# MPEGGroup/mpeg-pcc-tmc2

Hardware: AMD Instinct MI355X
Metric: encoder patch+image-gen frames/sec, longdress_vox10 32-frame GOF (higher is better)
Workload: dtype int32/f64

## Files before the change

### mpeg-pcc-tmc2_amd/csrc/api.cpp

```cpp
#include <algorithm>
#include <cstring>
#include <atomic>
#include <chrono>
#include <condition_variable>
#include <cstdarg>
#include <map>
#include <memory>
#include <mutex>

#include "internal.h"

extern char** environ;

namespace tmc2 {
int allowLargeLds( const void* kernel, size_t bytes, int device, size_t staticBytes ) {
  static std::mutex                                 lock;
  static std::map<std::pair<const void*, int>, int> granted;
  std::lock_guard<std::mutex>                       g( lock );
  int& have = granted[{kernel, device}];
  if ( int( bytes ) <= have ) return TMC2_OK;
  const int want = 160 * 1024 - int( ( staticBytes + 63 ) & ~size_t( 63 ) );
  if ( int( bytes ) > want ) {
    setError( "%zu bytes of dynamic LDS requested (+ %zu static): more than a gfx950 workgroup has", bytes, staticBytes );
    return TMC2_E_INVALID;
// ... 173 lines not shown
  (void)hipEventRecord( stages[id].pending.back().second, stream );
}
void tmc2_ctx::foldStage( StageTimer& t ) {
  for ( auto& pr : t.pending ) {
    float ms = 0.f;
    if ( hipEventSynchronize( pr.second ) == hipSuccess && hipEventElapsedTime( &ms, pr.first, pr.second ) == hipSuccess )
      t.ms += ms;
    freeEvents.push_back( pr.first );
    freeEvents.push_back( pr.second );
  }
  t.pending.clear();
}
void tmc2_ctx::stageAddHostMs( const char* name, double ms ) {
  for ( auto& s : stages )
    if ( s.name == name ) {
      s.ms += ms;
      s.calls++;
      return;
    }
  StageTimer t;
  t.name  = name;
  t.ms    = ms;
  t.calls = 1;
  stages.push_back( t );
}

extern "C" {

const char* tmc2_last_error( void ) { return g_lastError.c_str(); }

int tmc2_ctx_create( int device, tmc2_ctx** out ) {
  if ( !out ) return TMC2_E_INVALID;
  *out      = nullptr;
  int count = 0;
  if ( hipGetDeviceCount( &count ) != hipSuccess || count <= 0 ) {
    setError( "no HIP device visible: this library has no CPU path" );
    return TMC2_E_NO_DEVICE;
  }
  if ( device < 0 || device >= count ) {
    setError( "device %d out of range (%d visible)", device, count );
    return TMC2_E_INVALID;
  }
  TMC2_HIP( hipSetDevice( device ) );
  tmc2_ctx* c = new tmc2_ctx();
  c->device   = device;
  hipDeviceProp_t prop;
// ... 604 lines not shown
```

### mpeg-pcc-tmc2_amd/csrc/internal.h

```cpp
#pragma once
#include <hip/hip_runtime.h>

#include <algorithm>
#include <cstdint>
#include <cstdio>
#include <cstring>
#include <initializer_list>
#include <atomic>
#include <map>
#include <memory>
#include <mutex>
#include <optional>
#include <string>
#include <functional>
#include <vector>

#include "tmc2hip.h"

namespace tmc2 {

void setError( const char* fmt, ... );

#define TMC2_HIP( expr )                                                                        \
  do {                                                                                          \
// ... 237 lines not shown
  tmc2::DevBuf<uint32_t>        voxelBitmap;
  std::map<uint32_t, int>       kdLevelHint;
  struct ConstTable {
    tmc2::DevBuf<int> dev;
    std::vector<int>  host;
  };
  std::map<uint64_t, std::unique_ptr<ConstTable>> constTables;
  std::vector<std::unique_ptr<ConstTable>>        retiredTables;
  const int* constTable( uint64_t key, const std::vector<int>& host );
  uint32_t* mailbox = nullptr;
  static constexpr size_t kMailboxWords = 1024;
  volatile uint32_t* answerLine( int line ) const { return mailbox + size_t( line ) * 16; }
  enum { kAnswerRefineVoxels = 1, kAnswerPatchRound = 2, kAnswerRecon = 3, kAnswerOrientHead = 4, kAnswerTreeDepth = 5, kAnswerGeoError = 6, kAnswerAttrError = 7, kAnswerTreeLevels = 8 , kAnswerVoxelCount = 13 };
  std::map<std::string, std::string> options;
  mutable std::mutex                 optionsLock;
  std::shared_ptr<tmc2_host_gate>    hostGate;
  hipStream_t                   stream = nullptr;
  std::vector<tmc2::StageTimer> stages;
  std::vector<hipEvent_t>       freeEvents;
  bool                          timing = true;
  int                           cuCount = 256;
  void foldStage( tmc2::StageTimer& t );
  void stageAddHostMs( const char* name, double ms );

 private:
  friend struct tmc2::StageScope;
  int  stageBegin( const char* name );
  void stageEnd( int id );
};

namespace tmc2 {
struct StageScope {
  StageScope( tmc2_ctx* c, const char* name ) : ctx( c ), id( c->stageBegin( name ) ) {}
  StageScope( const StageScope& ) = delete;
  StageScope& operator=( const StageScope& ) = delete;
  ~StageScope() { end(); }
  void end() { ctx->stageEnd( id ), id = -1; }

 private:
  tmc2_ctx* ctx;
  int       id;
};
void destroyContextNow( tmc2_ctx* ctx );
struct FrameTicket {
  tmc2_ctx* ctx = nullptr;
  void      bind( tmc2_ctx* c ) {
// ... 207 lines not shown
```

### mpeg-pcc-tmc2_amd/csrc/kdtree_device.hip

```cpp
#include <algorithm>
#include <cstring>

#include "internal.h"

namespace tmc2 {
namespace {

constexpr uint32_t kNone      = 0xFFFFFFFFu;
constexpr int      kBlock     = 256;
constexpr int      kWaves     = kBlock / 64;
constexpr int      kScanTile  = kBlock * 8;
constexpr int      kLeafMax   = 10;
constexpr int      kMaxLevels = 64;

struct BuildSeg {
  uint32_t begin, end;
  uint32_t node, parent;
  int32_t  mn[3], mx[3];
  int16_t  lo[3], hi[3];
  uint8_t  side, pdim;
  uint8_t  split, cutDim;
  int32_t  cut;
  uint32_t mid;
  uint32_t slot;
};

struct RetiredSeg {
  uint32_t begin, end, node, level;
  int16_t  lo[3], hi[3];
  int32_t  root;
};

struct HugeSeg {
  uint32_t begin, end, node, level;
  int16_t  lo[3], hi[3];
  int32_t  root;
  int32_t  mn[3], mx[3];
};

struct BuildArgs {
  const Pt* pts;
  uint32_t  n, tiles;
  Pt*       P;
  uint32_t *perm, *seg;
  BuildSeg *segA, *segB;
  KdNode*   nodes;
  uint32_t *loc1, *loc2, *tile1, *tile2;
  uint32_t* counts;
  uint32_t* nodeCount;
  int32_t*  rootBox;
  uint32_t* levels;
  RetiredSeg* retired;
  uint32_t*   retiredCount;
  uint32_t*   bigCount;
  HugeSeg*    huge;
  uint32_t*   hugeCount;
  uint32_t    hugeMax;
  uint32_t    retireMax, splitMax;
  struct LvSeg *lvA, *lvB;
  uint16_t*   list;
  struct LvPartial* partial;
  unsigned long long* pieceProfile;
  uint32_t    decideRng;
  uint32_t*   finishDepth;
  uint32_t*   ticket;
  volatile uint32_t* hostSmall;
  volatile uint32_t* hostDepth;
};

__device__ __forceinline__ int coordOf( const Pt p, int d ) { return d == 0 ? p.x : ( d == 1 ? p.y : p.z ); }

struct SplitRule {
  int     dim;
  int32_t cut;
};
__device__ __forceinline__ SplitRule splitOf( const int16_t ( &lo )[3], const int16_t ( &hi )[3], const int32_t ( &mn )[3],
                                              const int32_t ( &mx )[3] ) {
  const int32_t maxSpan = max( int32_t( hi[0] ) - lo[0], max( int32_t( hi[1] ) - lo[1], int32_t( hi[2] ) - lo[2] ) );
  SplitRule     r;
  r.dim              = 0;
  int32_t bestSpread = -1;
#pragma unroll
  for ( int d = 0; d < 3; ++d ) {
    if ( double( int32_t( hi[d] ) - lo[d] ) > ( 1.0 - 0.00001 ) * double( maxSpan ) ) {
      const int32_t spread = mx[d] - mn[d];
      if ( spread > bestSpread ) {
        bestSpread = spread;
        r.dim      = d;
      }
    }
  }
// ... 166 lines not shown
          child[0].begin = q.begin, child[0].end = q.begin + idx, child[0].node = id0;
          child[1].begin = q.begin + idx, child[1].end = q.end, child[1].node = id0 + 1;
          for ( int c = 0; c < 2; ++c ) {
            child[c].depth = uint16_t( q.depth + 1 );
            for ( int d = 0; d < 3; ++d )
              child[c].lo[d] = lo[d], child[c].hi[d] = hi[d], child[c].mn[d] = int16_t( r[6 * c + d] ), child[c].mx[d] = int16_t( r[6 * c + 3 + d] );
          }
          const int16_t cut = int16_t( rule.cut );
          if ( rule.dim == 0 ) child[0].hi[0] = cut, child[1].lo[0] = cut;
          if ( rule.dim == 1 ) child[0].hi[1] = cut, child[1].lo[1] = cut;
          if ( rule.dim == 2 ) child[0].hi[2] = cut, child[1].lo[2] = cut;
          for ( int c = 0; c < 2; ++c ) {
            const uint32_t cc = child[c].end - child[c].begin, level = seg.level + child[c].depth;
            if ( cc <= uint32_t( kLeafMax ) ) {
              KdNode leaf;
              leaf.a = int32_t( seg.begin + child[c].begin ), leaf.b = int32_t( seg.begin + child[c].end ), leaf.divlow = leaf.divhigh = 0,
              leaf.dim = -1;
              a.nodes[child[c].node] = leaf;
              atomicMax( a.finishDepth, level + 1u );
            } else if ( cc <= a.retireMax ) {
              RetiredSeg rs;
              rs.begin = seg.begin + child[c].begin, rs.end = seg.begin + child[c].end, rs.node = child[c].node, rs.level = level, rs.root = 0;
              for ( int d = 0; d < 3; ++d ) rs.lo[d] = child[c].lo[d], rs.hi[d] = child[c].hi[d];
              a.retired[atomicAdd( a.retiredCount, 1u )] = rs;
            } else {
              sNode[cur ^ 1][sCount[cur ^ 1]++] = child[c];
            }
          }
        }
        __syncthreads();
      }
      if ( threadIdx.x == 0 ) sCount[cur] = 0;
      cur ^= 1;
      __syncthreads();
    }
  }
}

constexpr int      kPieceMax  = 4096;
constexpr int      kPieceRecs = kPieceMax / ( kLeafMax + 1 ) + 2;
constexpr uint16_t kNoRec     = 0xFFFFu;
constexpr uint32_t kNoKey     = 0xFFFFFFFFu;

struct alignas( 8 ) PieceRec {
  uint16_t begin, end;
  int16_t  cut;
  uint8_t  dim, unused0;
  uint16_t edge1, rb1;
  uint16_t edge2, rb2;
  uint16_t mid;
  uint16_t child[2];
  uint16_t unused1;
  uint32_t node;
  int32_t  lmax, rmin;
  int16_t  lo[3], hi[3];
  int32_t  mn[3], mx[3];
};
static_assert( sizeof( PieceRec ) == 72, "PieceRec layout" );
struct PieceHot0 {
  uint32_t be, dc;
};
struct PieceHot1 {
  uint32_t e1rb1, e2rb2;
// ... 115 lines not shown
  }
#pragma unroll
  for ( int off = 32; off > 0; off >>= 1 ) {
    mnx = min( mnx, __shfl_xor( mnx, off, 64 ) ), mny = min( mny, __shfl_xor( mny, off, 64 ) ), mnz = min( mnz, __shfl_xor( mnz, off, 64 ) );
    mxx = max( mxx, __shfl_xor( mxx, off, 64 ) ), mxy = max( mxy, __shfl_xor( mxy, off, 64 ) ), mxz = max( mxz, __shfl_xor( mxz, off, 64 ) );
  }
  if ( lane == 0 ) {
    int* w = blockRange + 6 * wave;
    w[0] = mnx, w[1] = mny, w[2] = mnz, w[3] = mxx, w[4] = mxy, w[5] = mxz;
  }
  __syncthreads();
  if ( threadIdx.x < 6 ) {
    int v = blockRange[threadIdx.x];
    for ( int w = 1; w < kWaves; ++w ) v = threadIdx.x < 3 ? min( v, blockRange[6 * w + threadIdx.x] ) : max( v, blockRange[6 * w + threadIdx.x] );
    int32_t* slot = threadIdx.x < 3 ? &a.lvA[0].mn[threadIdx.x] : &a.lvA[0].mx[threadIdx.x - 3];
    if ( threadIdx.x < 3 ) {
      if ( v < loadStaleOk( slot ) ) atomicMin( slot, v );
    } else {
      if ( v > loadStaleOk( slot ) ) atomicMax( slot, v );
    }
  }
}
__global__ void lvRootKernel( BuildArgs a ) {
  if ( threadIdx.x < kMaxLevels + 16 ) a.counts[threadIdx.x] = 0;
  __syncthreads();
  if ( threadIdx.x != 0 ) return;
  LvSeg r{};
  r.begin = 0, r.end = a.n, r.node = 0, r.parent = kNone;
  for ( int d = 0; d < 3; ++d ) r.mn[d] = 0x7FFFFFFF, r.mx[d] = int32_t( 0x80000000 );
  a.lvA[0]     = r;
  a.counts[0]  = 1;
  *a.nodeCount = 1;
}

constexpr int kDecideThreads = 1024;
constexpr int kDecideRng     = 2000;
__global__ __launch_bounds__( kDecideThreads ) void lvDecideKernel( BuildArgs a, uint32_t level ) {
  __shared__ uint32_t waveTot[kDecideThreads / 64];
  __shared__ uint32_t sCarry;
  __shared__ int32_t  sRng[kDecideRng][6];
  LvSeg*         cur   = ( level & 1 ) ? a.lvB : a.lvA;
  const uint32_t count = a.counts[level], nodeBase = *a.nodeCount;
  const int      lane = threadIdx.x & 63, wave = threadIdx.x >> 6;
  if ( threadIdx.x == 0 ) sCarry = 0;
  const bool inLds = level > 0 && count <= a.decideRng;
  if ( inLds ) {
    for ( uint32_t t = threadIdx.x; t < count * 6u; t += kDecideThreads ) sRng[t / 6u][t % 6u] = ( t % 6u ) < 3u ? 0x7FFFFFFF : int32_t( 0x80000000 );
// ... 37 lines not shown
        if ( inLds ) mn[d] = min( mn[d], sRng[s][d] ), mx[d] = max( mx[d], sRng[s][3 + d] );
        lo[d] = root ? mn[d] : int32_t( q->lo[d] );
        hi[d] = root ? mx[d] : int32_t( q->hi[d] );
      }
      if ( root ) {
        for ( int d = 0; d < 3; ++d ) a.rootBox[d] = mn[d], a.rootBox[3 + d] = mx[d];
      } else {
        const int pd = q->pdim;
        if ( q->side == 0 )
          a.nodes[q->parent].divlow = int16_t( pd == 0 ? mx[0] : ( pd == 1 ? mx[1] : mx[2] ) );
        else
          a.nodes[q->parent].divhigh = int16_t( pd == 0 ? mn[0] : ( pd == 1 ? mn[1] : mn[2] ) );
      }
      const uint32_t cnt = q->end - q->begin;
      if ( cnt <= uint32_t( kLeafMax ) ) {
        KdNode nd;
        nd.a = int32_t( q->begin ), nd.b = int32_t( q->end ), nd.divlow = nd.divhigh = 0, nd.dim = -1;
        a.nodes[q->node] = nd;
      } else if ( cnt <= a.retireMax ) {
        RetiredSeg r;
        r.begin = q->begin, r.end = q->end, r.node = q->node, r.level = level;
        r.root  = root ? 1 : 0;
        for ( int d = 0; d < 3; ++d ) r.lo[d] = q->lo[d], r.hi[d] = q->hi[d];
        a.retired[atomicAdd( a.retiredCount, 1u )] = r;
      } else if ( cnt <= a.hugeMax ) {
        HugeSeg r;
        r.begin = q->begin, r.end = q->end, r.node = q->node, r.level = level;
        r.root  = root ? 1 : 0;
        for ( int d = 0; d < 3; ++d ) r.lo[d] = q->lo[d], r.hi[d] = q->hi[d], r.mn[d] = mn[d], r.mx[d] = mx[d];
        a.huge[atomicAdd( a.hugeCount, 1u )] = r;
      } else {
        const int32_t maxSpan = max( hi[0] - lo[0], max( hi[1] - lo[1], hi[2] - lo[2] ) );
        const double  limit   = ( 1.0 - 0.00001 ) * double( maxSpan );
        int           dim     = 0;
        int32_t       best    = -1;
        if ( double( hi[0] - lo[0] ) > limit && mx[0] - mn[0] > best ) best = mx[0] - mn[0], dim = 0;
        if ( double( hi[1] - lo[1] ) > limit && mx[1] - mn[1] > best ) best = mx[1] - mn[1], dim = 1;
        if ( double( hi[2] - lo[2] ) > limit && mx[2] - mn[2] > best ) best = mx[2] - mn[2], dim = 2;
        const int32_t l = dim == 0 ? lo[0] : ( dim == 1 ? lo[1] : lo[2] ), h = dim == 0 ? hi[0] : ( dim == 1 ? hi[1] : hi[2] );
        const int32_t lowest = dim == 0 ? mn[0] : ( dim == 1 ? mn[1] : mn[2] ), highest = dim == 0 ? mx[0] : ( dim == 1 ? mx[1] : mx[2] );
        const int32_t cut = min( max( ( l + h ) / 2, lowest ), highest );
        q->cutInfo = ( uint32_t( cut ) & 0xFFFFu ) | ( uint32_t( dim ) << 16 ) | ( 1u << 24 );
        if ( root )
          for ( int d = 0; d < 3; ++d ) q->lo[d] = int16_t( mn[d] ), q->hi[d] = int16_t( mx[d] );
        split = 1;
      }
      if ( !split ) q->cutInfo = 0;
// ... 4 lines not shown
      const uint32_t t = __shfl_up( inc, off, 64 );
      if ( lane >= off ) inc += t;
    }
    if ( lane == 63 ) waveTot[wave] = inc;
    __syncthreads();
    uint32_t before = sCarry, all = 0;
    for ( int w = 0; w < kDecideThreads / 64; ++w ) {
      all += waveTot[w];
      before += w < wave ? waveTot[w] : 0u;
    }
    const uint32_t rank = before + inc - split;
    if ( split ) q->slot = 2u * rank, q->childNode = nodeBase + 2u * rank;
    __syncthreads();
    if ( threadIdx.x == 0 ) sCarry += all;
    __syncthreads();
  }
  if ( threadIdx.x == 0 ) {
    a.counts[level + 1] = 2u * sCarry;
    *a.nodeCount        = nodeBase + 2u * sCarry;
  }
  if ( a.hostSmall ) {
    if ( threadIdx.x == 0 ) __threadfence();
    __syncthreads();
    if ( threadIdx.x < kMaxLevels + 16 ) a.hostSmall[threadIdx.x] = __hip_atomic_load( &a.counts[threadIdx.x], __ATOMIC_RELAXED, __HIP_MEMORY_SCOPE_AGENT );
  }
}

template <bool FIRST>
__global__ __launch_bounds__( kBlock ) void lvFlagKernel( BuildArgs a, uint32_t level ) {
  __shared__ uint32_t waveSum[kWaves];
  const uint32_t n = a.n, tiles = a.tiles;
  const int      lane = threadIdx.x & 63, wave = threadIdx.x >> 6;
  LvSeg*         cur   = ( level & 1 ) ? a.lvB : a.lvA;
  LvSeg*         next  = ( level & 1 ) ? a.lvA : a.lvB;
  const uint32_t count = a.counts[level];
  uint32_t*      loc   = FIRST ? a.loc1 : a.loc2;
  uint32_t*      tile  = FIRST ? a.tile1 : a.tile2;
  if ( !FIRST ) {
    for ( uint32_t s = blockIdx.x * blockDim.x + threadIdx.x; s < count; s += gridDim.x * blockDim.x ) {
      const LvSeg* q = cur + s;
      if ( !( q->cutInfo >> 24 ) ) continue;
      for ( int c = 0; c < 2; ++c )
        for ( int d = 0; d < 3; ++d ) next[q->slot + c].mn[d] = 0x7FFFFFFF, next[q->slot + c].mx[d] = int32_t( 0x80000000 );
    }
  }
  for ( uint32_t t = blockIdx.x; t < tiles; t += gridDim.x ) {
    const uint32_t base = t * kScanTile + threadIdx.x * 8;
// ... 210 lines not shown
          }
          for ( int k = 0; k < 6; ++k ) accV[k] = accSlot == kNone ? x[k] : ( ( k % 3 ) == 1 ? pkMax( accV[k], x[k] ) : pkMin( accV[k], x[k] ) );
          accSlot = slot;
        }
      }
      __syncthreads();
      continue;
    }
    if ( moved ) lvReport( next + slot + 1u, pkLo( A2 ), pkHi( A2 ), pkLo( C2 ), pkLo( A2 ), pkHi( A2 ), pkLo( C2 ) );
    if ( waveSegMinMaxPacked( key, A, B, C, lane ) )
      lvReport( next + key, pkLo( A ), pkHi( A ), pkLo( C ), pkLo( B ), pkHi( B ), ~pkHi( C ) );
  }
  __syncthreads();
  if ( threadIdx.x == 0 ) {
    LvPartial pt;
    pt.slot = accSlot, pt.unused = 0;
    for ( int k = 0; k < 6; ++k ) pt.v[k] = accV[k];
    a.partial[c0 / kChunk] = pt;
  }
  __syncthreads();
  }
}

constexpr size_t kPieceLdsBytes = size_t( kPieceMax ) * ( sizeof( Pt ) + 4 + 2 + 2 + 2 ) + 16 + 2 * size_t( kPieceRecs ) * sizeof( PieceRec );

constexpr int kPiecePer = 4;
template <bool PROFILE = false>
__global__ __launch_bounds__( kPieceMax / kPiecePer ) void pieceKernel( BuildArgs a ) {
  unsigned long long profLast = 0, prof[12] = {0, 0, 0, 0, 0, 0, 0, 0, 0, 0, 0, 0};
#define PIECE_MARK( k )                                        \
  if ( PROFILE && threadIdx.x == 0 ) {                         \
    const unsigned long long now_ = wall_clock64();            \
    prof[k] += now_ - profLast, profLast = now_;               \
  }
  constexpr int K = kPiecePer, THREADS = kPieceMax / K, WAVES = THREADS / 64;
  extern __shared__ __align__( 16 ) unsigned char pieceLds[];
  Pt*       P     = reinterpret_cast<Pt*>( pieceLds );
  uint32_t* perm  = reinterpret_cast<uint32_t*>( P + kPieceMax );
  uint16_t* pre   = reinterpret_cast<uint16_t*>( perm + kPieceMax );
  uint16_t* lst   = pre + kPieceMax + 8;
  uint16_t* segOf = lst + kPieceMax;
  PieceRec* recs  = reinterpret_cast<PieceRec*>( segOf + kPieceMax );
  __shared__ __align__( 16 ) uint32_t sWave[2][WAVES];
  __shared__ uint32_t sCount[2], sNodeBase, sDepth;
  const int      lane = threadIdx.x & 63, tid = threadIdx.x;
  const uint32_t total = *a.retiredCount;
  const uint32_t p0    = uint32_t( tid ) * K;
  for ( uint32_t s = blockIdx.x; s < total; s += gridDim.x ) {
    const RetiredSeg seg = a.retired[s];
    const uint32_t   cnt = seg.end - seg.begin;
    uint32_t idPending   = 0;
    if ( tid == 0 ) idPending = atomicAdd( a.nodeCount, 2u );
    pieceBarrier();
    for ( uint32_t i = tid; i < uint32_t( kPieceMax ); i += THREADS ) {
      if ( i < cnt ) {
        P[i]     = a.P[seg.begin + i];
        perm[i]  = a.perm[seg.begin + i];
        segOf[i] = 0;
      } else {
        segOf[i] = kNoRec;
      }
    }
    if ( tid == 0 ) {
      PieceRec r{};
      r.begin = 0, r.end = uint16_t( cnt ), r.node = seg.node;
      for ( int d = 0; d < 3; ++d ) r.lo[d] = seg.lo[d], r.hi[d] = seg.hi[d], r.mn[d] = 0x7FFFFFFF, r.mx[d] = int32_t( 0x80000000 );
      recs[0]   = r;
      sCount[0] = 1, sCount[1] = 0, sDepth = 0;
    }
    pieceBarrier();
    {
      uint32_t A = pk2( 0x7FFF, 0x7FFF ), B = pk2( -0x8000, -0x8000 ), C = pk2( 0x7FFF, 0x7FFF );
      bool     any = false;
#pragma unroll
      for ( int k = 0; k < K; ++k ) {
        const uint32_t p = p0 + k;
        if ( p < cnt ) {
// ... 2 lines not shown
          any = true;
        }
      }
      if ( waveSegMinMaxPacked( any ? 0u : kNoKey, A, B, C, lane ) ) {
        ldsMin( &recs[0].mn[0], pkLo( A ) ), ldsMin( &recs[0].mn[1], pkHi( A ) ), ldsMin( &recs[0].mn[2], pkLo( C ) );
        ldsMax( &recs[0].mx[0], pkLo( B ) ), ldsMax( &recs[0].mx[1], pkHi( B ) ), ldsMax( &recs[0].mx[2], ~pkHi( C ) );
      }
    }
    pieceBarrier();
    if ( seg.root != 0 && tid == 0 ) {
      for ( int d = 0; d < 3; ++d ) {
        recs[0].lo[d] = int16_t( recs[0].mn[d] ), recs[0].hi[d] = int16_t( recs[0].mx[d] );
        a.rootBox[d] = recs[0].mn[d], a.rootBox[3 + d] = recs[0].mx[d];
      }
    }
    if ( PROFILE && threadIdx.x == 0 ) profLast = wall_clock64();
    uint32_t deepest  = 0;
    uint32_t prevBase = 0, prevCount = 0;
    int      cur      = 0;
    for ( uint32_t depth = 0;; ++depth ) {
      pieceBarrier();
      PIECE_MARK( 0 )
      const uint32_t nc = sCount[cur];
      PieceRec*      R  = recs + cur * kPieceRecs;
      PieceRec*      RN = recs + ( cur ^ 1 ) * kPieceRecs;
      for ( uint32_t r = tid; r < prevCount; r += THREADS ) {
        const PieceRec* q = RN + r;
        KdNode          nd;
        nd.a = int32_t( prevBase + 2u * r ), nd.b = int32_t( prevBase + 2u * r + 1u ), nd.divlow = int16_t( q->lmax ), nd.divhigh = int16_t( q->rmin ),
        nd.dim = q->dim;
        a.nodes[q->node] = nd;
      }
      if ( nc == 0 ) break;
      if ( seg.level + depth >= uint32_t( kMaxLevels ) - 2u ) {
        if ( tid == 0 ) atomicMax( a.finishDepth, 0x10000u );
        break;
      }
      if ( tid == 0 ) sNodeBase = idPending, sCount[cur ^ 1] = 0;
      for ( uint32_t r = tid; r < nc; r += THREADS ) {
        PieceRec*     q   = R + r;
        const int32_t lo0 = q->lo[0], lo1 = q->lo[1], lo2 = q->lo[2], hi0 = q->hi[0], hi1 = q->hi[1], hi2 = q->hi[2];
        const int32_t mn0 = q->mn[0], mn1 = q->mn[1], mn2 = q->mn[2], mx0 = q->mx[0], mx1 = q->mx[1], mx2 = q->mx[2];
        const int32_t maxSpan = max( hi0 - lo0, max( hi1 - lo1, hi2 - lo2 ) );
        const double  limit   = ( 1.0 - 0.00001 ) * double( maxSpan );
        int           dim     = 0;
        int32_t       best    = -1;
        if ( double( hi0 - lo0 ) > limit && mx0 - mn0 > best ) best = mx0 - mn0, dim = 0;
        if ( double( hi1 - lo1 ) > limit && mx1 - mn1 > best ) best = mx1 - mn1, dim = 1;
// ... 27 lines not shown
          }
        }
      }
      uint32_t f1 = 0;
      if ( waveLive ) {
        Pt x[K];
#pragma unroll
        for ( int k = 0; k < K; k += 2 ) *reinterpret_cast<uint4*>( &x[k] ) = *reinterpret_cast<const uint4*>( P + p0 + k );
#pragma unroll
        for ( int k = 0; k < K; ++k ) {
          const int d = int( ( dc[k] >> 16 ) & 0xFFu ), c = int( int16_t( dc[k] & 0xFFFFu ) );
          const int v = int( int16_t( __builtin_bit_cast( uint64_t, x[k] ) >> ( 16 * d ) ) );
          if ( rec[k] != kNoRec && v >= c ) f1 |= 1u << k;
        }
      }
      uint32_t preA[K + 1];
      {
        uint32_t at = pieceScan<WAVES>( uint32_t( __popc( f1 ) ), sWave[0] );
        uint16_t out[K];
#pragma unroll
        for ( int k = 0; k < K; ++k ) preA[k] = at, out[k] = uint16_t( at ), at += ( f1 >> k ) & 1u;
        preA[K] = at;
        *reinterpret_cast<uint2*>( pre + p0 ) = *reinterpret_cast<const uint2*>( out );
        if ( tid == THREADS - 1 ) pre[kPieceMax] = uint16_t( at );
      }
      pieceBarrier();
      PIECE_MARK( 2)
      uint32_t edge1[K], rb1[K];
#pragma unroll
      for ( int k = 0; k < K; ++k ) {
        edge1[k] = rb1[k] = 0;
        if ( !waveLive || rec[k] == kNoRec ) continue;
        if ( k > 0 && rec[k] == rec[k - 1] ) {
          edge1[k] = edge1[k - 1], rb1[k] = rb1[k - 1];
        } else {
          const uint32_t b = be[k] & 0xFFFFu, e = be[k] >> 16, rb = pre[b], re = pre[e];
          edge1[k] = b + ( ( e - b ) - ( re - rb ) ), rb1[k] = rb | ( re << 16 );
        }
        const uint32_t p = p0 + k, b = be[k] & 0xFFFFu, e = be[k] >> 16;
        if ( p >= edge1[k] && !( ( f1 >> k ) & 1u ) ) lst[b + ( ( e - p - 1u ) - ( ( rb1[k] >> 16 ) - preA[k + 1] ) )] = uint16_t( p );
        if ( p == b ) *reinterpret_cast<uint32_t*>( &R[rec[k]].edge1 ) = edge1[k] | ( ( rb1[k] & 0xFFFFu ) << 16 );
      }
      pieceBarrier();
      PIECE_MARK( 3)
#pragma unroll
      for ( int k = 0; k < K; ++k ) {
        const uint32_t p = p0 + k;
// ... 5 lines not shown
        }
      }
      pieceBarrier();
      PIECE_MARK( 4)
      uint32_t f2 = 0;
      if ( waveLive ) {
        Pt x[K];
#pragma unroll
        for ( int k = 0; k < K; k += 2 ) *reinterpret_cast<uint4*>( &x[k] ) = *reinterpret_cast<const uint4*>( P + p0 + k );
#pragma unroll
        for ( int k = 0; k < K; ++k ) {
          const int d = int( ( dc[k] >> 16 ) & 0xFFu ), c = int( int16_t( dc[k] & 0xFFFFu ) );
          const int v = int( int16_t( __builtin_bit_cast( uint64_t, x[k] ) >> ( 16 * d ) ) );
          if ( rec[k] != kNoRec && p0 + k >= edge1[k] && v > c ) f2 |= 1u << k;
        }
      }
      {
        uint32_t at = pieceScan<WAVES>( uint32_t( __popc( f2 ) ), sWave[1] );
        uint16_t out[K];
#pragma unroll
        for ( int k = 0; k < K; ++k ) preA[k] = at, out[k] = uint16_t( at ), at += ( f2 >> k ) & 1u;
        preA[K] = at;
        *reinterpret_cast<uint2*>( pre + p0 ) = *reinterpret_cast<const uint2*>( out );
        if ( tid == THREADS - 1 ) pre[kPieceMax] = uint16_t( at );
      }
      pieceBarrier();
      PIECE_MARK( 5)
      const uint32_t base = sNodeBase;
      for ( uint32_t r = tid; r < nc; r += THREADS ) {
        PieceRec*      q  = R + r;
        const uint32_t b = q->begin, e = q->end, e1 = q->edge1, rb2 = pre[e1], re2 = pre[e];
        const uint32_t e2   = e1 + ( ( e - e1 ) - ( re2 - rb2 ) );
        const uint32_t n    = e - b, half = n / 2, lim1 = e1 - b, lim2 = e2 - b;
        const uint32_t idx  = lim1 > half ? lim1 : ( lim2 < half ? lim2 : half );
        const uint32_t mid  = b + idx;
        const uint32_t id0  = base + 2u * r;
        const int      dim  = q->dim;
        const int16_t  cut  = q->cut;
        q->edge2 = uint16_t( e2 ), q->rb2 = uint16_t( rb2 ), q->mid = uint16_t( mid );
        q->lmax = int32_t( 0x80000000 ), q->rmin = 0x7FFFFFFF;
#pragma unroll
        for ( int c = 0; c < 2; ++c ) {
          const uint32_t cb = c ? mid : b, ce = c ? e : mid;
          if ( ce - cb <= uint32_t( kLeafMax ) ) {
            KdNode leaf;
            leaf.a = int32_t( seg.begin + cb ), leaf.b = int32_t( seg.begin + ce ), leaf.divlow = leaf.divhigh = 0, leaf.dim = -1;
            a.nodes[id0 + c] = leaf;
// ... 134 lines not shown
  const uint32_t n = uint32_t( n64 );
  tree.n           = n64;
  tree.depth       = 0;
  for ( int d = 0; d < 3; ++d ) tree.lo[d] = tree.hi[d] = 0;
  if ( n == 0 ) return TMC2_OK;
  hipStream_t    s       = ctx->stream;
  const uint32_t tiles   = ( n + kScanTile - 1 ) / kScanTile;
  const size_t   maxSegs = 2 * ( size_t( n ) / ( kLeafMax + 1 ) + 1 ) + 2;
  const size_t   maxNode = 2 * size_t( n ) + 2;
  TMC2_TRY( tree.ptsTree.alloc( n ) );
  TMC2_TRY( tree.perm.alloc( n ) );
  TMC2_TRY( tree.nodes.alloc( maxNode ) );
  DevBuf<uint32_t>   d_work, d_small;
  DevBuf<BuildSeg>   d_segs;
  DevBuf<RetiredSeg> d_retired;
  const size_t       maxRetired = size_t( n ) / ( kLeafMax + 1 ) + 2;
  TMC2_TRY( d_retired.alloc( maxRetired ) );
  DevBuf<HugeSeg> d_huge;
  TMC2_TRY( d_huge.alloc( size_t( n ) / ( kPieceMax + 1 ) + 2 ) );
  const auto     hugeEnv = ctxOption( ctx, "KD_HUGEMAX" );
  const uint32_t hugeMax = std::min<uint32_t>( kHugeLimit, std::max<uint32_t>( kPieceMax, hugeEnv ? uint32_t( atoi( hugeEnv->c_str() ) ) : 16384u ) );
  TMC2_TRY( d_work.alloc( 3 * size_t( n ) + 2 * ( size_t( tiles ) + 1 ) ) );
  TMC2_TRY( d_segs.alloc( 2 * maxSegs ) );
  TMC2_TRY( d_small.alloc( kMaxLevels + 16 ) );
  static_assert( kMaxLevels + 16 <= 128, "lvRootKernel clears the counters with one workgroup of 128" );
  BuildArgs a;
  a.pts = d_pts, a.n = n, a.tiles = tiles, a.P = tree.ptsTree.p, a.perm = tree.perm.p;
  a.seg = d_work.p, a.loc1 = d_work.p + n, a.loc2 = d_work.p + 2 * size_t( n );
  a.tile1 = d_work.p + 3 * size_t( n ), a.tile2 = a.tile1 + tiles + 1;
  a.segA = d_segs.p, a.segB = d_segs.p + maxSegs, a.nodes = tree.nodes.p;
  a.counts    = d_small.p;
  a.nodeCount = d_small.p + kMaxLevels + 1;
  a.levels    = d_small.p + kMaxLevels + 2;
  a.rootBox   = reinterpret_cast<int32_t*>( d_small.p + kMaxLevels + 8 );
  a.retired      = d_retired.p;
  a.retiredCount = d_small.p + kMaxLevels + 3;
  a.finishDepth  = d_small.p + kMaxLevels + 4;
  a.ticket       = d_small.p + kMaxLevels + 5;
  a.bigCount     = d_small.p + kMaxLevels + 6;
  a.huge         = d_huge.p;
  a.hugeCount    = d_small.p + kMaxLevels + 7;
  a.hugeMax      = hugeMax;
  a.hostSmall    = nullptr;
  a.hostDepth    = ctx->answerLine( tmc2_ctx::kAnswerTreeDepth );
  a.retireMax    = uint32_t( kPieceMax );
  a.splitMax     = uint32_t( kPieceMax );
  const dim3 blk( kBlock ), grdE( std::max<uint32_t>( 1u, ( n + 2 * kBlock - 1 ) / ( 2 * kBlock ) ) ), grdT( tiles );
  const dim3 grdL( std::max<uint32_t>( 1u, ( n + kLandBlock * kLandRounds - 1 ) / ( kLandBlock * kLandRounds ) ) );
  const size_t sumsLds = ( size_t( tiles ) + 1 ) * 4;
  if ( sumsLds > 48 * 1024 ) {
    setError( "kdtree: %u points -- the level passes hold one word per 2 048-point tile in LDS (at most 25 M points)", n );
    return TMC2_E_UNSUPPORTED;
  }
  DevBuf<LvSeg>    d_lv;
  DevBuf<uint16_t> d_list;
  DevBuf<LvPartial> d_partial;
  const size_t     maxLv = 2 * ( size_t( n ) / ( size_t( kPieceMax ) + 1 ) + 2 );
  TMC2_TRY( d_lv.alloc( 2 * maxLv ) );
  TMC2_TRY( d_list.alloc( size_t( tiles ) * kScanTile ) );
  TMC2_TRY( d_partial.alloc( size_t( n ) / ( kLandBlock * kLandRounds ) + 2 ) );
  a.lvA = d_lv.p, a.lvB = d_lv.p + maxLv, a.list = d_list.p, a.partial = d_partial.p;
  const auto decideOpt = ctxOption( ctx, "KD_DECIDE" );
  a.decideRng = decideOpt && ( *decideOpt )[0] == 'g' ? 0u : uint32_t( kDecideRng );
  hipLaunchKernelGGL( lvRootKernel, dim3( 1 ), dim3( 128 ), 0, s, a );
  hipLaunchKernelGGL( lvInitKernel, dim3( std::min<uint32_t>( grdE.x, 1024u ) ), blk, 0, s, a );
  hipLaunchKernelGGL( lvDecideKernel, dim3( 1 ), dim3( kDecideThreads ), 0, s, a, 0u );
  uint32_t out[kMaxLevels + 16];
  int      found = -1;
  int& hint = ctx->kdLevelHint[( n >> 15 ) * 2u + 1u];
  for ( uint32_t level = 0; level < uint32_t( kMaxLevels ) && found < 0; ) {
    uint32_t chunkEnd = level + 1;
    if ( level == 0 && hint > 0 ) {
      chunkEnd = uint32_t( std::min( hint, kMaxLevels ) );
    } else {
      while ( chunkEnd < uint32_t( kMaxLevels ) && ( uint64_t( hugeMax ) << std::min<uint32_t>( chunkEnd - 1, 40 ) ) < n ) ++chunkEnd;
      if ( chunkEnd == level + 1 ) chunkEnd = std::min<uint32_t>( level + 2, kMaxLevels );
    }
    volatile uint32_t* hostSmall = ctx->answerLine( tmc2_ctx::kAnswerTreeLevels );
    for ( ; level < chunkEnd; ++level ) {
      hipLaunchKernelGGL( lvFlagKernel<true>, grdT, blk, 0, s, a, level );
      hipLaunchKernelGGL( lvSwapOneKernel, grdE, blk, sumsLds, s, a, level );
      hipLaunchKernelGGL( lvFlagKernel<false>, grdT, blk, 0, s, a, level );
      hipLaunchKernelGGL( lvSwapTwoKernel, grdL, dim3( kLandBlock ), sumsLds, s, a, level );
      BuildArgs ad = a;
      if ( level + 1 == chunkEnd ) ad.hostSmall = hostSmall;
      hipLaunchKernelGGL( lvDecideKernel, dim3( 1 ), dim3( kDecideThreads ), 0, s, ad, level + 1u );
    }
    TMC2_HIP( hipGetLastError() );
    TMC2_HIP( hipStreamSynchronize( s ) );
    for ( int w = 0; w < kMaxLevels + 16; ++w ) out[w] = hostSmall[w];
    for ( uint32_t l = 0; l <= level && l <= uint32_t( kMaxLevels ); ++l )
      if ( out[l] == 0 ) {
        found = int( l );
        break;
      }
  }
  if ( found < 0 ) {
    setError( "kdtree: more than %d levels", kMaxLevels - 1 );
    return TMC2_E_UNSUPPORTED;
  }
  tree.depth = found;
  hint       = std::max( found, 1 );
  const int32_t* box = reinterpret_cast<const int32_t*>( out + kMaxLevels + 8 );
  for ( int d = 0; d < 3; ++d ) tree.lo[d] = box[d], tree.hi[d] = box[3 + d];
  const uint32_t hugeSegs = out[kMaxLevels + 7];
  if ( hugeSegs )
    hipLaunchKernelGGL( hugeSegmentsKernel, dim3( std::min<uint32_t>( hugeSegs, 4u * uint32_t( ctx->cuCount ) ) ), dim3( 64 * kHugeWaves ), 0, s, a );
  const uint32_t retired = out[kMaxLevels + 3] + hugeSegs * ( 2u * hugeMax / uint32_t( kPieceMax ) );
  if ( retired ) {
    const dim3 grid( std::min<uint32_t>( retired, 8u * uint32_t( ctx->cuCount ) ) ), block( kPieceMax / kPiecePer );
    if ( ctxOption( ctx, "KD_PIECE_PROFILE" ) ) {
      DevBuf<unsigned long long> d_prof;
      TMC2_TRY( d_prof.alloc( 16 ) );
      TMC2_HIP( hipMemsetAsync( d_prof.p, 0, 16 * 8, s ) );
      a.pieceProfile = d_prof.p;
      TMC2_TRY( allowLargeLds( reinterpret_cast<const void*>( pieceKernel<true> ), kPieceLdsBytes, ctx->device, 256 ) );
      hipLaunchKernelGGL( pieceKernel<true>, grid, block, kPieceLdsBytes, s, a );
      unsigned long long h[16];
      TMC2_HIP( hipMemcpyAsync( h, d_prof.p, sizeof( h ), hipMemcpyDeviceToHost, s ) );
      TMC2_HIP( hipStreamSynchronize( s ) );
      static const char* what[8] = {"landing of the previous depth", "node records + split rules", "first flags + prefix sum", "first publish",
                                    "first swaps", "second flags + prefix sum", "children + second publish", "second swaps"};
      fprintf( stderr, "pieceKernel: %llu pieces, us per piece between the barriers of its depths (thread 0 of each workgroup):", h[8] );
      for ( int k = 0; k < 8; ++k ) fprintf( stderr, " %s %.1f |", what[k], 0.01 * double( h[k] ) / double( std::max<unsigned long long>( h[8], 1 ) ) );
      fprintf( stderr, "\n" );
    } else {
      TMC2_TRY( allowLargeLds( reinterpret_cast<const void*>( pieceKernel<> ), kPieceLdsBytes, ctx->device, 256 ) );
      hipLaunchKernelGGL( pieceKernel<>, grid, block, kPieceLdsBytes, s, a );
    }
    TMC2_HIP( hipGetLastError() );
    TMC2_HIP( hipStreamSynchronize( s ) );
    const uint32_t fin = *a.hostDepth;
    if ( fin >= uint32_t( kMaxLevels ) ) {
      setError( "kdtree: more than %d levels", kMaxLevels - 1 );
      return TMC2_E_UNSUPPORTED;
    }
    tree.depth = std::max( tree.depth, int( fin ) );
  }
  return TMC2_OK;
}

}
```

Baseline: 198.9.

## Bin retired kd-tree pieces by size and launch per-capacity piece kernels

Retired segments are now sorted into three size classes (up to 1024, 2048 and 4096 points). Each class gets its own pieceKernel instantiation, sized so that smaller classes use less LDS and fewer threads, which lets two or four workgroups share a CU. Workgroups take pieces through an atomic ticket instead of a grid-stride loop. The aim is to stop small pieces from occupying a full 4096-capacity workgroup and to balance work dynamically. The cost is extra kernel launches, a class-list buffer, and more atomics per piece.

```diff
diff --git a/mpeg-pcc-tmc2_amd/csrc/api.cpp b/mpeg-pcc-tmc2_amd/csrc/api.cpp
--- a/mpeg-pcc-tmc2_amd/csrc/api.cpp
+++ b/mpeg-pcc-tmc2_amd/csrc/api.cpp
@@ -219,6 +219,17 @@
   t.name  = name;
   t.ms    = ms;
   t.calls = 1;
+  stages.push_back( t );
+}
+void tmc2_ctx::stageAddCalls( const char* name, long calls ) {
+  for ( auto& s : stages )
+    if ( s.name == name ) {
+      s.calls += calls;
+      return;
+    }
+  StageTimer t;
+  t.name  = name;
+  t.calls = calls;
   stages.push_back( t );
 }
 
diff --git a/mpeg-pcc-tmc2_amd/csrc/internal.h b/mpeg-pcc-tmc2_amd/csrc/internal.h
--- a/mpeg-pcc-tmc2_amd/csrc/internal.h
+++ b/mpeg-pcc-tmc2_amd/csrc/internal.h
@@ -283,6 +283,7 @@
   int                           cuCount = 256;
   void foldStage( tmc2::StageTimer& t );
   void stageAddHostMs( const char* name, double ms );
+  void stageAddCalls( const char* name, long calls );
 
  private:
   friend struct tmc2::StageScope;
diff --git a/mpeg-pcc-tmc2_amd/csrc/kdtree_device.hip b/mpeg-pcc-tmc2_amd/csrc/kdtree_device.hip
--- a/mpeg-pcc-tmc2_amd/csrc/kdtree_device.hip
+++ b/mpeg-pcc-tmc2_amd/csrc/kdtree_device.hip
@@ -12,6 +12,17 @@
 constexpr int      kScanTile  = kBlock * 8;
 constexpr int      kLeafMax   = 10;
 constexpr int      kMaxLevels = 64;
+constexpr int      kPieceMax  = 4096;
+constexpr int      kPieceClasses = 3;
+constexpr int      kSmallHost  = kMaxLevels + 16;
+constexpr int      kSmallWords = kMaxLevels + 24;
+enum : int {
+  kWordNodeCount = kMaxLevels + 1, kWordRetired, kWordFinishDepth, kWordTicket, kWordHugeCount,
+  kWordClassCount,
+  kWordRootBox     = kSmallHost - 6,
+  kWordClassTicket = kSmallHost
+};
+static_assert( kWordClassCount + kPieceClasses <= kWordRootBox && kWordClassTicket + kPieceClasses <= kSmallWords, "counter block" );
 
 struct BuildSeg {
   uint32_t begin, end;
@@ -49,10 +60,12 @@
   uint32_t* counts;
   uint32_t* nodeCount;
   int32_t*  rootBox;
-  uint32_t* levels;
   RetiredSeg* retired;
   uint32_t*   retiredCount;
-  uint32_t*   bigCount;
+  uint32_t*   classCount;
+  uint32_t*   classList;
+  uint32_t    classStride;
+  uint32_t*   classTicket;
   HugeSeg*    huge;
   uint32_t*   hugeCount;
   uint32_t    hugeMax;
@@ -67,6 +80,14 @@
   volatile uint32_t* hostSmall;
   volatile uint32_t* hostDepth;
 };
+
+__device__ __forceinline__ void retirePiece( const BuildArgs& a, const RetiredSeg& r ) {
+  const uint32_t at = atomicAdd( a.retiredCount, 1u );
+  a.retired[at]     = r;
+  const uint32_t cnt = r.end - r.begin;
+  const int      c   = cnt <= uint32_t( kPieceMax >> 2 ) ? 0 : ( cnt <= uint32_t( kPieceMax >> 1 ) ? 1 : 2 );
+  a.classList[size_t( c ) * a.classStride + atomicAdd( a.classCount + c, 1u )] = at;
+}
 
 __device__ __forceinline__ int coordOf( const Pt p, int d ) { return d == 0 ? p.x : ( d == 1 ? p.y : p.z ); }
 
@@ -279,7 +300,7 @@
               RetiredSeg rs;
               rs.begin = seg.begin + child[c].begin, rs.end = seg.begin + child[c].end, rs.node = child[c].node, rs.level = level, rs.root = 0;
               for ( int d = 0; d < 3; ++d ) rs.lo[d] = child[c].lo[d], rs.hi[d] = child[c].hi[d];
-              a.retired[atomicAdd( a.retiredCount, 1u )] = rs;
+              retirePiece( a, rs );
             } else {
               sNode[cur ^ 1][sCount[cur ^ 1]++] = child[c];
             }
@@ -294,8 +315,7 @@
   }
 }
 
-constexpr int      kPieceMax  = 4096;
-constexpr int      kPieceRecs = kPieceMax / ( kLeafMax + 1 ) + 2;
+constexpr int pieceRecs( int cap ) { return cap / ( kLeafMax + 1 ) + 2; }
 constexpr uint16_t kNoRec     = 0xFFFFu;
 constexpr uint32_t kNoKey     = 0xFFFFFFFFu;
 
@@ -457,7 +477,7 @@
   }
 }
 __global__ void lvRootKernel( BuildArgs a ) {
-  if ( threadIdx.x < kMaxLevels + 16 ) a.counts[threadIdx.x] = 0;
+  if ( threadIdx.x < kSmallWords ) a.counts[threadIdx.x] = 0;
   __syncthreads();
   if ( threadIdx.x != 0 ) return;
   LvSeg r{};
@@ -541,7 +561,7 @@
         r.begin = q->begin, r.end = q->end, r.node = q->node, r.level = level;
         r.root  = root ? 1 : 0;
         for ( int d = 0; d < 3; ++d ) r.lo[d] = q->lo[d], r.hi[d] = q->hi[d];
-        a.retired[atomicAdd( a.retiredCount, 1u )] = r;
+        retirePiece( a, r );
       } else if ( cnt <= a.hugeMax ) {
         HugeSeg r;
         r.begin = q->begin, r.end = q->end, r.node = q->node, r.level = level;
@@ -592,7 +612,7 @@
   if ( a.hostSmall ) {
     if ( threadIdx.x == 0 ) __threadfence();
     __syncthreads();
-    if ( threadIdx.x < kMaxLevels + 16 ) a.hostSmall[threadIdx.x] = __hip_atomic_load( &a.counts[threadIdx.x], __ATOMIC_RELAXED, __HIP_MEMORY_SCOPE_AGENT );
+    if ( threadIdx.x < kSmallHost ) a.hostSmall[threadIdx.x] = __hip_atomic_load( &a.counts[threadIdx.x], __ATOMIC_RELAXED, __HIP_MEMORY_SCOPE_AGENT );
   }
 }
 
@@ -849,37 +869,48 @@
   }
 }
 
-constexpr size_t kPieceLdsBytes = size_t( kPieceMax ) * ( sizeof( Pt ) + 4 + 2 + 2 + 2 ) + 16 + 2 * size_t( kPieceRecs ) * sizeof( PieceRec );
+constexpr size_t pieceLdsBytes( int cap ) { return size_t( cap ) * ( sizeof( Pt ) + 4 + 2 + 2 + 2 ) + 16 + 2 * size_t( pieceRecs( cap ) ) * sizeof( PieceRec ); }
+constexpr size_t kCuLdsBytes = 160 * 1024, kPieceStatic = 256;
+static_assert( pieceLdsBytes( kPieceMax ) + kPieceStatic <= kCuLdsBytes, "a piece of kPieceMax points fits a CU" );
+static_assert( 2 * ( pieceLdsBytes( kPieceMax >> 1 ) + kPieceStatic ) <= kCuLdsBytes, "two workgroups of the 2 048 instance per CU" );
+static_assert( 4 * ( pieceLdsBytes( kPieceMax >> 2 ) + kPieceStatic ) <= kCuLdsBytes, "four workgroups of the 1 024 instance per CU" );
 
 constexpr int kPiecePer = 4;
-template <bool PROFILE = false>
-__global__ __launch_bounds__( kPieceMax / kPiecePer ) void pieceKernel( BuildArgs a ) {
+template <int CAP, bool PROFILE = false>
+__global__ __launch_bounds__( CAP / kPiecePer ) void pieceKernel( BuildArgs a ) {
+  static_assert( CAP == kPieceMax || CAP == kPieceMax >> 1 || CAP == kPieceMax >> 2, "one instance per capacity class" );
+  constexpr int CLS = CAP == kPieceMax ? 2 : ( CAP == kPieceMax >> 1 ? 1 : 0 ), RECS = pieceRecs( CAP );
   unsigned long long profLast = 0, prof[12] = {0, 0, 0, 0, 0, 0, 0, 0, 0, 0, 0, 0};
 #define PIECE_MARK( k )                                        \
   if ( PROFILE && threadIdx.x == 0 ) {                         \
     const unsigned long long now_ = wall_clock64();            \
     prof[k] += now_ - profLast, profLast = now_;               \
   }
-  constexpr int K = kPiecePer, THREADS = kPieceMax / K, WAVES = THREADS / 64;
+  constexpr int K = kPiecePer, THREADS = CAP / K, WAVES = THREADS / 64;
+  static_assert( WAVES % 4 == 0, "pieceScan reads the wavefront totals four at a time" );
   extern __shared__ __align__( 16 ) unsigned char pieceLds[];
   Pt*       P     = reinterpret_cast<Pt*>( pieceLds );
-  uint32_t* perm  = reinterpret_cast<uint32_t*>( P + kPieceMax );
-  uint16_t* pre   = reinterpret_cast<uint16_t*>( perm + kPieceMax );
-  uint16_t* lst   = pre + kPieceMax + 8;
-  uint16_t* segOf = lst + kPieceMax;
-  PieceRec* recs  = reinterpret_cast<PieceRec*>( segOf + kPieceMax );
+  uint32_t* perm  = reinterpret_cast<uint32_t*>( P + CAP );
+  uint16_t* pre   = reinterpret_cast<uint16_t*>( perm + CAP );
+  uint16_t* lst   = pre + CAP + 8;
+  uint16_t* segOf = lst + CAP;
+  PieceRec* recs  = reinterpret_cast<PieceRec*>( segOf + CAP );
   __shared__ __align__( 16 ) uint32_t sWave[2][WAVES];
-  __shared__ uint32_t sCount[2], sNodeBase, sDepth;
+  __shared__ uint32_t sCount[2], sNodeBase, sDepth, sPiece;
   const int      lane = threadIdx.x & 63, tid = threadIdx.x;
-  const uint32_t total = *a.retiredCount;
+  const uint32_t total = a.classCount[CLS];
+  const uint32_t* mine = a.classList + size_t( CLS ) * a.classStride;
   const uint32_t p0    = uint32_t( tid ) * K;
-  for ( uint32_t s = blockIdx.x; s < total; s += gridDim.x ) {
-    const RetiredSeg seg = a.retired[s];
+  for ( ;; ) {
+    if ( tid == 0 ) sPiece = atomicAdd( a.classTicket + CLS, 1u );
+    pieceBarrier();
+    const uint32_t t = sPiece;
+    if ( t >= total ) break;
+    const RetiredSeg seg = a.retired[mine[t]];
     const uint32_t   cnt = seg.end - seg.begin;
     uint32_t idPending   = 0;
     if ( tid == 0 ) idPending = atomicAdd( a.nodeCount, 2u );
-    pieceBarrier();
-    for ( uint32_t i = tid; i < uint32_t( kPieceMax ); i += THREADS ) {
+    for ( uint32_t i = tid; i < uint32_t( CAP ); i += THREADS ) {
       if ( i < cnt ) {
         P[i]     = a.P[seg.begin + i];
         perm[i]  = a.perm[seg.begin + i];
@@ -928,8 +959,8 @@
       pieceBarrier();
       PIECE_MARK( 0 )
       const uint32_t nc = sCount[cur];
-      PieceRec*      R  = recs + cur * kPieceRecs;
-      PieceRec*      RN = recs + ( cur ^ 1 ) * kPieceRecs;
+      PieceRec*      R  = recs + cur * RECS;
+      PieceRec*      RN = recs + ( cur ^ 1 ) * RECS;
       for ( uint32_t r = tid; r < prevCount; r += THREADS ) {
         const PieceRec* q = RN + r;
         KdNode          nd;
@@ -1003,7 +1034,7 @@
         for ( int k = 0; k < K; ++k ) preA[k] = at, out[k] = uint16_t( at ), at += ( f1 >> k ) & 1u;
         preA[K] = at;
         *reinterpret_cast<uint2*>( pre + p0 ) = *reinterpret_cast<const uint2*>( out );
-        if ( tid == THREADS - 1 ) pre[kPieceMax] = uint16_t( at );
+        if ( tid == THREADS - 1 ) pre[CAP] = uint16_t( at );
       }
       pieceBarrier();
       PIECE_MARK( 2)
@@ -1055,7 +1086,7 @@
         for ( int k = 0; k < K; ++k ) preA[k] = at, out[k] = uint16_t( at ), at += ( f2 >> k ) & 1u;
         preA[K] = at;
         *reinterpret_cast<uint2*>( pre + p0 ) = *reinterpret_cast<const uint2*>( out );
-        if ( tid == THREADS - 1 ) pre[kPieceMax] = uint16_t( at );
+        if ( tid == THREADS - 1 ) pre[CAP] = uint16_t( at );
       }
       pieceBarrier();
       PIECE_MARK( 5)
@@ -1236,24 +1267,28 @@
   const uint32_t hugeMax = std::min<uint32_t>( kHugeLimit, std::max<uint32_t>( kPieceMax, hugeEnv ? uint32_t( atoi( hugeEnv->c_str() ) ) : 16384u ) );
   TMC2_TRY( d_work.alloc( 3 * size_t( n ) + 2 * ( size_t( tiles ) + 1 ) ) );
   TMC2_TRY( d_segs.alloc( 2 * maxSegs ) );
-  TMC2_TRY( d_small.alloc( kMaxLevels + 16 ) );
-  static_assert( kMaxLevels + 16 <= 128, "lvRootKernel clears the counters with one workgroup of 128" );
+  TMC2_TRY( d_small.alloc( kSmallWords ) );
+  static_assert( kSmallWords <= 128, "lvRootKernel clears the counters with one workgroup of 128" );
+  DevBuf<uint32_t> d_classList;
+  TMC2_TRY( d_classList.alloc( size_t( kPieceClasses ) * maxRetired ) );
   BuildArgs a;
   a.pts = d_pts, a.n = n, a.tiles = tiles, a.P = tree.ptsTree.p, a.perm = tree.perm.p;
   a.seg = d_work.p, a.loc1 = d_work.p + n, a.loc2 = d_work.p + 2 * size_t( n );
   a.tile1 = d_work.p + 3 * size_t( n ), a.tile2 = a.tile1 + tiles + 1;
   a.segA = d_segs.p, a.segB = d_segs.p + maxSegs, a.nodes = tree.nodes.p;
   a.counts    = d_small.p;
-  a.nodeCount = d_small.p + kMaxLevels + 1;
-  a.levels    = d_small.p + kMaxLevels + 2;
-  a.rootBox   = reinterpret_cast<int32_t*>( d_small.p + kMaxLevels + 8 );
+  a.nodeCount = d_small.p + kWordNodeCount;
+  a.rootBox   = reinterpret_cast<int32_t*>( d_small.p + kWordRootBox );
   a.retired      = d_retired.p;
-  a.retiredCount = d_small.p + kMaxLevels + 3;
-  a.finishDepth  = d_small.p + kMaxLevels + 4;
-  a.ticket       = d_small.p + kMaxLevels + 5;
-  a.bigCount     = d_small.p + kMaxLevels + 6;
+  a.retiredCount = d_small.p + kWordRetired;
+  a.classCount   = d_small.p + kWordClassCount;
+  a.classList    = d_classList.p;
+  a.classStride  = uint32_t( maxRetired );
+  a.classTicket  = d_small.p + kWordClassTicket;
+  a.finishDepth  = d_small.p + kWordFinishDepth;
+  a.ticket       = d_small.p + kWordTicket;
   a.huge         = d_huge.p;
-  a.hugeCount    = d_small.p + kMaxLevels + 7;
+  a.hugeCount    = d_small.p + kWordHugeCount;
   a.hugeMax      = hugeMax;
   a.hostSmall    = nullptr;
   a.hostDepth    = ctx->answerLine( tmc2_ctx::kAnswerTreeDepth );
@@ -1279,7 +1314,7 @@
   hipLaunchKernelGGL( lvRootKernel, dim3( 1 ), dim3( 128 ), 0, s, a );
   hipLaunchKernelGGL( lvInitKernel, dim3( std::min<uint32_t>( grdE.x, 1024u ) ), blk, 0, s, a );
   hipLaunchKernelGGL( lvDecideKernel, dim3( 1 ), dim3( kDecideThreads ), 0, s, a, 0u );
-  uint32_t out[kMaxLevels + 16];
+  uint32_t out[kSmallHost];
   int      found = -1;
   int& hint = ctx->kdLevelHint[( n >> 15 ) * 2u + 1u];
   for ( uint32_t level = 0; level < uint32_t( kMaxLevels ) && found < 0; ) {
@@ -1302,7 +1337,7 @@
     }
     TMC2_HIP( hipGetLastError() );
     TMC2_HIP( hipStreamSynchronize( s ) );
-    for ( int w = 0; w < kMaxLevels + 16; ++w ) out[w] = hostSmall[w];
+    for ( int w = 0; w < kSmallHost; ++w ) out[w] = hostSmall[w];
     for ( uint32_t l = 0; l <= level && l <= uint32_t( kMaxLevels ); ++l )
       if ( out[l] == 0 ) {
         found = int( l );
@@ -1315,21 +1350,48 @@
   }
   tree.depth = found;
   hint       = std::max( found, 1 );
-  const int32_t* box = reinterpret_cast<const int32_t*>( out + kMaxLevels + 8 );
+  const int32_t* box = reinterpret_cast<const int32_t*>( out + kWordRootBox );
   for ( int d = 0; d < 3; ++d ) tree.lo[d] = box[d], tree.hi[d] = box[3 + d];
-  const uint32_t hugeSegs = out[kMaxLevels + 7];
+  const uint32_t hugeSegs = out[kWordHugeCount];
   if ( hugeSegs )
     hipLaunchKernelGGL( hugeSegmentsKernel, dim3( std::min<uint32_t>( hugeSegs, 4u * uint32_t( ctx->cuCount ) ) ), dim3( 64 * kHugeWaves ), 0, s, a );
-  const uint32_t retired = out[kMaxLevels + 3] + hugeSegs * ( 2u * hugeMax / uint32_t( kPieceMax ) );
-  if ( retired ) {
-    const dim3 grid( std::min<uint32_t>( retired, 8u * uint32_t( ctx->cuCount ) ) ), block( kPieceMax / kPiecePer );
-    if ( ctxOption( ctx, "KD_PIECE_PROFILE" ) ) {
-      DevBuf<unsigned long long> d_prof;
+  uint32_t classGrid[kPieceClasses];
+  int      lastClass = -1;
+  for ( int c = 0; c < kPieceClasses; ++c ) {
+    const uint32_t cap = uint32_t( kPieceMax ) >> ( kPieceClasses - 1 - c ), above = c == 0 ? uint32_t( kLeafMax ) : cap / 2u;
+    const uint64_t most = uint64_t( out[kWordClassCount + c] ) + uint64_t( hugeSegs ) * ( hugeMax / ( above + 1u ) );
+    const uint32_t resident = uint32_t( ctx->cuCount ) * ( uint32_t( kPieceMax ) / cap );
+    classGrid[c] = uint32_t( std::min<uint64_t>( most, resident ) );
+    if ( classGrid[c] && lastClass < 0 ) lastClass = c;
+  }
+  if ( lastClass >= 0 ) {
+    const bool profile = ctxOption( ctx, "KD_PIECE_PROFILE" ).has_value();
+    DevBuf<unsigned long long> d_prof;
+    if ( profile ) {
       TMC2_TRY( d_prof.alloc( 16 ) );
       TMC2_HIP( hipMemsetAsync( d_prof.p, 0, 16 * 8, s ) );
       a.pieceProfile = d_prof.p;
-      TMC2_TRY( allowLargeLds( reinterpret_cast<const void*>( pieceKernel<true> ), kPieceLdsBytes, ctx->device, 256 ) );
-      hipLaunchKernelGGL( pieceKernel<true>, grid, block, kPieceLdsBytes, s, a );
+    }
+    for ( int c = kPieceClasses - 1; c >= 0; --c ) {
+      if ( !classGrid[c] ) continue;
+      BuildArgs ac = a;
+      if ( c != lastClass ) ac.hostDepth = nullptr;
+      const dim3 grid( classGrid[c] );
+#define TMC2_PIECE_LAUNCH( CAP )                                                                                                   \
+  {                                                                                                                                \
+    const void* fn = profile ? reinterpret_cast<const void*>( pieceKernel<CAP, true> ) : reinterpret_cast<const void*>( pieceKernel<CAP> ); \
+    TMC2_TRY( allowLargeLds( fn, pieceLdsBytes( CAP ), ctx->device, kPieceStatic ) );                                              \
+    if ( profile )                                                                                                                 \
+      hipLaunchKernelGGL( ( pieceKernel<CAP, true> ), grid, dim3( CAP / kPiecePer ), pieceLdsBytes( CAP ), s, ac );                \
+    else                                                                                                                           \
+      hipLaunchKernelGGL( ( pieceKernel<CAP> ), grid, dim3( CAP / kPiecePer ), pieceLdsBytes( CAP ), s, ac );                      \
+  }
+      if ( c == 2 ) TMC2_PIECE_LAUNCH( kPieceMax )
+      if ( c == 1 ) TMC2_PIECE_LAUNCH( kPieceMax / 2 )
+      if ( c == 0 ) TMC2_PIECE_LAUNCH( kPieceMax / 4 )
+#undef TMC2_PIECE_LAUNCH
+    }
+    if ( profile ) {
       unsigned long long h[16];
       TMC2_HIP( hipMemcpyAsync( h, d_prof.p, sizeof( h ), hipMemcpyDeviceToHost, s ) );
       TMC2_HIP( hipStreamSynchronize( s ) );
@@ -1338,9 +1400,10 @@
       fprintf( stderr, "pieceKernel: %llu pieces, us per piece between the barriers of its depths (thread 0 of each workgroup):", h[8] );
       for ( int k = 0; k < 8; ++k ) fprintf( stderr, " %s %.1f |", what[k], 0.01 * double( h[k] ) / double( std::max<unsigned long long>( h[8], 1 ) ) );
       fprintf( stderr, "\n" );
-    } else {
-      TMC2_TRY( allowLargeLds( reinterpret_cast<const void*>( pieceKernel<> ), kPieceLdsBytes, ctx->device, 256 ) );
-      hipLaunchKernelGGL( pieceKernel<>, grid, block, kPieceLdsBytes, s, a );
+      static const char* className[kPieceClasses] = {"kdtree_pieces_cap1024", "kdtree_pieces_cap2048", "kdtree_pieces_cap4096"};
+      for ( int c = 0; c < kPieceClasses; ++c ) ctx->stageAddCalls( className[c], long( out[kWordClassCount + c] ) );
+      ctx->stageAddCalls( "kdtree_pieces_retired", long( out[kWordRetired] ) );
+      ctx->stageAddCalls( "kdtree_pieces_finished", long( h[8] ) );
     }
     TMC2_HIP( hipGetLastError() );
     TMC2_HIP( hipStreamSynchronize( s ) );
```

Result: slower. 195.7 (-1.6%).
